# yangao07/abPOA

Measured on NVIDIA H100. Metric: GCUPS (DP cells/s), global/convex 10 kbp, higher is better.
Workload: dtype int16 (packed int16x2 DPX arithmetic; int32 kernel only as overflow fallback)

## Files before the change

### abpoa_b200/csrc/poa_kernels.cu

```cuda
#include <cuda_runtime.h>
#include <stdint.h>
#include <algorithm>
#include "poa_device.cuh"
#include "poa_chain.cuh"

#define FULL 0xffffffffu
#define NEG POA_NEG32

enum { LG = 0, AG = 1, CG = 2 };
enum { GLOBAL = 0, LOCAL = 1, EXTEND = 2 };

#define OP_M   0x1
#define OP_E1  0x2
#define OP_E2  0x4
#define OP_E   0x6
#define OP_F1  0x8
#define OP_F2  0x10
#define OP_F   0x18
#define OP_ALL 0x1f

__device__ __forceinline__ void ld8(const int16_t *p, int v[8]) {
    const uint4 u = *reinterpret_cast<const uint4 *>(p);
    v[0] = (int)(short)(u.x & 0xffff); v[1] = ((int)u.x) >> 16;
    v[2] = (int)(short)(u.y & 0xffff); v[3] = ((int)u.y) >> 16;
// ... 697 lines not shown
            int E1o[8], E2o[8];
            int lmax = NEG, lfirst = -1, llast = -1;
#pragma unroll
            for (int c = 0; c < 8; ++c) {
                const int j = g * 8 + c, jr = j - jbase;
                if (GAP == LG) {
                    x1 = max(x1, a1[c]);
                    int h = max(x1 - e1 * jr, NEG);
                    if (MODE == LOCAL) h = max(h, zr);
                    if (lgx) {
                        const int v = j >> xs;
                        const bool keep = active && j >= beg && j <= ((((end >> xs) + 1) << xs) - 1) &&
                                          (v <= lgx_v1 || (v == lgx_v1 + 1 && !(j & 1)));
                        H[c] = keep ? h : NEG;
                    } else
                    H[c] = inb[c] ? h : NEG;
                } else {
                    const int f1 = max(x1 - e1 * (jr - 1), NEG);
                    x1 = max(x1, a1[c]);
                    Fa[c] = f1;
                    if (GAP == AG) {
                        const int t = max(M[c], X1[c]);
                        int h = max(t, f1);
                        if (MODE == LOCAL) h = max(h, zr);
                        const bool from_t = (h == t);
                        E1o[c] = from_t ? max(X1[c] - e1, h - oe1) : (MODE == LOCAL ? 0 : NEG);
                        H[c] = h;
                    } else {
                        const int f2 = max(x2 - e2 * (jr - 1), NEG);
                        x2 = max(x2, a2[c]);
                        Fb[c] = f2;
                        int h = max(T[c], max(f1, f2));
                        if (MODE == LOCAL) h = max(h, zr);
                        int eo1 = max(X1[c] - e1, h - oe1), eo2 = max(X2[c] - e2, h - oe2);
                        if (MODE == LOCAL) { eo1 = max(eo1, zr); eo2 = max(eo2, zr); }
                        E1o[c] = eo1; E2o[c] = eo2; H[c] = h;
                    }
                    if (!inb[c]) { H[c] = NEG; E1o[c] = NEG; if (GAP == CG) E2o[c] = NEG; }
                }
                if (inb[c]) {
                    if (H[c] > lmax) { lmax = H[c]; lfirst = llast = j; }
                    else if (H[c] == lmax) llast = j;
                }
            }

            if (active) {
                const int rel = g - g0;
                if (rel < ring_groups) {
                    ST *rq = ringp + (size_t)rel * POA_GROUP;
                    st8(rq, H);
                    if (GAP != LG) st8(rq + ring_cells, E1o);
                    if (GAP == CG) st8(rq + 2 * ring_cells, E2o);
                }
                ST *q = rowp + (size_t)rel * POA_GROUP;
                st8(q, H);
                if (GAP != LG) { st8(q + (size_t)PL::E1 * ngrp * POA_GROUP, E1o); st8(q + (size_t)PL::F1 * ngrp * POA_GROUP, Fa); }
                if (GAP == CG) { st8(q + (size_t)PL::E2 * ngrp * POA_GROUP, E2o); st8(q + (size_t)PL::F2 * ngrp * POA_GROUP, Fb); }
            }

            if (banded || MODE != GLOBAL) {
                const int pm = __reduce_max_sync(FULL, lmax);
                const unsigned bm = __ballot_sync(FULL, lmax == pm && lfirst >= 0);
                if (bm) {
                    const int pl = __shfl_sync(FULL, lfirst, __ffs(bm) - 1);
                    const int pr = __shfl_sync(FULL, llast, 31 - __clz(bm));
                    if (pm > row_max) { row_max = pm; row_left = pl; row_right = pr; }
                    else if (pm == row_max) row_right = pr;
                }
            }
        }
        if (lane == 0) {
            PoaRowInfo ri; ri.beg = beg; ri.end = end; ri.left = row_left; ri.right = row_right;
            ring_info[i & rmask] = ri; ring_off[i & rmask] = my_off;
            rowinfo[i] = ri; { PoaRowOff z; z.off = my_off; z.p0 = mypred; *reinterpret_cast<uint2 *>(rowoff + i) = make_uint2(z.off, (unsigned)z.p0); }
        }
        if (MODE == LOCAL) {
            if (row_max > best_score) { best_score = row_max; best_i = i; best_j = row_left; }
        } else if (MODE == EXTEND) {
            if (row_max > best_score) { best_score = row_max; best_i = i; best_j = row_right; best_row = i; }
            else if (prm->zdrop > 0) {
                const int delta = jv.remain(best_row) - rem;
                if (best_score - row_max > prm->zdrop + e1 * abs(delta - (row_right - best_j))) stop = true;
            }
        }
        __syncwarp();
        }
        pb = pe; pe = n_pe; rbase = n_rbase; rem = n_rem; mypred = n_mypred; myps = n_myps;
    }

    if (MODE == GLOBAL) {
        const int sb = jv.predoff(n_rows - 1), sn = jv.predoff(n_rows) - sb;
        for (int k = 0; k < sn; ++k) {
            const int prow = jv.pred[sb + k];
            const PoaRowInfo pi = rowinfo[prow];
            const int endc = qlen > pi.end ? pi.end : qlen;
            const int pg0 = ((pi.beg >> xs) << xs) >> 3;
            const int v = (endc >= pi.beg) ? (int)planes[(size_t)rowoff[prow].off * POA_GROUP + (endc - pg0 * 8)] : NEG;
            if (v > best_score) { best_score = v; best_i = prow; best_j = endc; }
        }
    }
    res.best_score = best_score; res.best_i = best_i; res.best_j = best_j;
    res.cells = cells; res.max_band = max_band; res.plane_units_used = cursor;
    const long long clk1 = clock64();
    res.fwd_clk = clk1 - clk0;
    if (lane == 0) *jd.result = res;
    __syncwarp();
    if (prm->ret_cigar) {
        poa_backtrack<GAP, ST, MODE>(jv, jd, prm, mat_s, lane, best_i, best_j, *jd.result, xs);
        if (lane == 0) jd.result->bt_clk = clock64() - clk1;
    }
    if (lane == 0) signal_done(jd);
}

#ifdef POA_KPROF
#define KP_DECL long long kp[6] = {0,0,0,0,0,0}; long long kp_t = clock64(); int kdiag[4] = {0,0,0,0};
#define KP(n) { const long long t_ = clock64(); kp[n] += t_ - kp_t; kp_t = t_; }
#define KP_OUT(res) { for (int z_ = 0; z_ < 6; ++z_) (res).prof[z_] = kp[z_]; for (int z_ = 0; z_ < 4; ++z_) (res).diag[z_] = kdiag[z_]; }
#else
#define KP_DECL
#define KP(n)
#define KP_OUT(res)
#endif
#define NEGP (-30000)
#define NEGP2 0x8AD08AD0u

__device__ __forceinline__ unsigned pk(int lo, int hi) { return ((unsigned)lo & 0xffffu) | ((unsigned)hi << 16); }
__device__ __forceinline__ int lo16(unsigned v) { return (int)(short)(v & 0xffffu); }
__device__ __forceinline__ int hi16(unsigned v) { return ((int)v) >> 16; }
__device__ __forceinline__ unsigned bc_hi(unsigned v) { return __byte_perm(v, v, 0x3232); }
__device__ __forceinline__ unsigned sh1(unsigned prev, unsigned cur) { return __byte_perm(prev, cur, 0x5432); }

__device__ __forceinline__ void lane_excl_prefix(const unsigned a[4], unsigned xb, unsigned P[4]) {
    unsigned inc[4];
#pragma unroll
    for (int k = 0; k < 4; ++k) inc[k] = __vmaxs2(a[k], __byte_perm(a[k], NEGP2, 0x1054));
    inc[1] = __vmaxs2(inc[1], bc_hi(inc[0]));
    inc[2] = __vmaxs2(inc[2], bc_hi(inc[1]));
    inc[3] = __vmaxs2(inc[3], bc_hi(inc[2]));
    P[0] = __vmaxs2(sh1(xb, inc[0]), xb);
    P[1] = __vmaxs2(sh1(inc[0], inc[1]), xb);
    P[2] = __vmaxs2(sh1(inc[1], inc[2]), xb);
    P[3] = __vmaxs2(sh1(inc[2], inc[3]), xb);
}
__device__ __forceinline__ int lane_max8(const unsigned a[4]) {
    const unsigned m = __vmaxs2(__vmaxs2(a[0], a[1]), __vmaxs2(a[2], a[3]));
    return max(lo16(m), hi16(m));
}

struct P16Consts {
    unsigned K1[4], K2[4];
    unsigned KF1[4], KF2[4];
    unsigned KLG[4];
    unsigned NE1, NOE1, NE2, NOE2;
};
static inline unsigned pk_host(int lo, int hi) { return ((unsigned)lo & 0xffffu) | ((unsigned)hi << 16); }
static P16Consts make_p16_consts(int e1, int oe1, int e2, int oe2) {
    P16Consts c;
    for (int k = 0; k < 4; ++k) {
        c.K1[k] = pk_host(e1 * (2 * k), e1 * (2 * k + 1)); c.K2[k] = pk_host(e2 * (2 * k), e2 * (2 * k + 1));
        c.KF1[k] = pk_host(-(oe1 + e1 * (2 * k - 1)), -(oe1 + e1 * (2 * k))); c.KF2[k] = pk_host(-(oe2 + e2 * (2 * k - 1)), -(oe2 + e2 * (2 * k)));
        c.KLG[k] = pk_host(-e1 * (2 * k), -e1 * (2 * k + 1));
    }
    c.NE1 = pk_host(-e1, -e1); c.NOE1 = pk_host(-oe1, -oe1); c.NE2 = pk_host(-e2, -e2); c.NOE2 = pk_host(-oe2, -oe2);
    return c;
}

struct P16Smem {
    int *mat_s; uint4 *cap_lo, *cap_hi, *ring_meta; int16_t *ring_data;
};
__device__ __forceinline__ P16Smem p16_smem_init(uint8_t *dyn_smem, const PoaParamsDev *prm, int ring_rows, int lane) {
    P16Smem sm;
    sm.mat_s = reinterpret_cast<int *>(dyn_smem);
    sm.cap_lo = reinterpret_cast<uint4 *>(dyn_smem + POA_MAX_M * POA_MAX_M * sizeof(int));
    sm.cap_hi = sm.cap_lo + 9;
    sm.ring_meta = sm.cap_hi + 9;
    sm.ring_data = reinterpret_cast<int16_t *>(sm.ring_meta + ring_rows);
    const int m = prm->m;
    for (int t = lane; t < m * m; t += 32) sm.mat_s[t] = prm->mat[t];
    if (lane < 9) {
        unsigned lo[4], hi[4];
#pragma unroll
        for (int k = 0; k < 4; ++k) {
            lo[k] = pk(2 * k < lane ? NEGP : 32767, 2 * k + 1 < lane ? NEGP : 32767);
            hi[k] = pk(2 * k >= 8 - lane ? NEGP : 32767, 2 * k + 1 >= 8 - lane ? NEGP : 32767);
        }
        sm.cap_lo[lane] = make_uint4(lo[0], lo[1], lo[2], lo[3]);
        sm.cap_hi[lane] = make_uint4(hi[0], hi[1], hi[2], hi[3]);
    }
    __syncwarp();
    return sm;
}

template <int GAP, int MODE>
__device__ __forceinline__ void p16_cells(const P16Consts &kc, const unsigned CLO[4], const unsigned CAP[4], const unsigned S[4],
                                          unsigned M[4], const unsigned X1[4], const unsigned X2[4], int jr0, int e1, int oe1, int e2, int oe2,
                                          unsigned zr2, int lane, int &carry1, int &carry2,
                                          unsigned H[4], unsigned F1[4], unsigned F2[4], unsigned E1o[4], unsigned E2o[4]) {
    unsigned T[4];
#pragma unroll
    for (int k = 0; k < 4; ++k) {
        const unsigned hm = __viaddmax_s16x2(M[k], S[k], NEGP2);
        M[k] = __vmins2(hm, CLO[k]);
        if (GAP == LG) T[k] = __vmins2(__vmaxs2(hm, X1[k]), CLO[k]);
        else if (GAP == AG) T[k] = M[k];
        else T[k] = __vmins2(__vimax3_s16x2(hm, X1[k], X2[k]), CLO[k]);
    }
    unsigned a1[4], a2[4];
#pragma unroll
    for (int k = 0; k < 4; ++k) { a1[k] = __vadd2(T[k], kc.K1[k]); if (GAP == CG) a2[k] = __vadd2(T[k], kc.K2[k]); }
    const int off1 = e1 * jr0 - (GAP == LG ? 0 : oe1), off2 = e2 * jr0 - oe2;
    int tot1, tot2 = 0;
    int x1 = max(warp_excl_max(lane_max8(a1) + off1, lane, tot1), carry1);
    carry1 = max(carry1, tot1);
    const int xl1 = min(max(x1 - off1, NEGP), 32767);
    unsigned P1[4], P2[4];
    lane_excl_prefix(a1, pk(xl1, xl1), P1);
    if (GAP == CG) {
        int x2 = max(warp_excl_max(lane_max8(a2) + off2, lane, tot2), carry2);
        carry2 = max(carry2, tot2);
        const int xl2 = min(max(x2 - off2, NEGP), 32767);
        lane_excl_prefix(a2, pk(xl2, xl2), P2);
    }
#pragma unroll
    for (int k = 0; k < 4; ++k) {
        if (GAP == LG) {
            unsigned h = __viaddmax_s16x2(__vmaxs2(P1[k], a1[k]), kc.KLG[k], NEGP2);
            if (MODE == LOCAL) h = __vmaxs2(h, zr2);
            H[k] = __vmins2(h, CAP[k]);
        } else {
            F1[k] = __viaddmax_s16x2(P1[k], kc.KF1[k], NEGP2);
            if (GAP == AG) {
                const unsigned t = __vmaxs2(M[k], X1[k]);
                unsigned fz = F1[k];
                if (MODE == LOCAL) fz = __vmaxs2(fz, zr2);
                const unsigned h = __vmaxs2(t, fz);
                const unsigned from_t = __vcmpges2(t, fz);
                const unsigned ev = __viaddmax_s16x2(X1[k], kc.NE1, __viaddmax_s16x2(h, kc.NOE1, NEGP2));
                const unsigned alt = (MODE == LOCAL) ? zr2 : NEGP2;
                E1o[k] = __vmins2((ev & from_t) | (alt & ~from_t), CAP[k]);
                H[k] = __vmins2(h, CAP[k]);
            } else {
                F2[k] = __viaddmax_s16x2(P2[k], kc.KF2[k], NEGP2);
                unsigned h = __vimax3_s16x2(T[k], F1[k], F2[k]);
                if (MODE == LOCAL) h = __vmaxs2(h, zr2);
                unsigned eo1 = __viaddmax_s16x2(X1[k], kc.NE1, __viaddmax_s16x2(h, kc.NOE1, NEGP2));
                unsigned eo2 = __viaddmax_s16x2(X2[k], kc.NE2, __viaddmax_s16x2(h, kc.NOE2, NEGP2));
                if (MODE == LOCAL) { eo1 = __vmaxs2(eo1, zr2); eo2 = __vmaxs2(eo2, zr2); }
                H[k] = __vmins2(h, CAP[k]); E1o[k] = __vmins2(eo1, CAP[k]); E2o[k] = __vmins2(eo2, CAP[k]);
            }
        }
    }
}

template <int GAP>
__device__ __forceinline__ uint2 p16_fbits(const P16Consts &kc, const unsigned H[4], const unsigned F1[4], const unsigned F2[4],
                                           const unsigned CLO[4], const unsigned CAP[4], bool left_in, int lane, bool more,
                                           unsigned &lh, unsigned &lf1, unsigned &lf2) {
    const unsigned hl = __shfl_up_sync(FULL, H[3], 1), f1l = __shfl_up_sync(FULL, F1[3], 1);
    unsigned f2l = 0u;
    if (GAP == CG) f2l = __shfl_up_sync(FULL, F2[3], 1);
    const unsigned hp = lane == 0 ? lh : hl, f1p = lane == 0 ? lf1 : f1l, f2p = lane == 0 ? lf2 : f2l;
    const unsigned clp = left_in ? 0x7fff0000u : 0u;
    unsigned v[4];
#pragma unroll
    for (int k = 0; k < 4; ++k) {
        const unsigned inb = __vcmpeq2(CAP[k], 0x7fff7fffu);
        const unsigned inl = inb & __vcmpeq2(sh1(k ? CLO[k - 1] : clp, CLO[k]), 0x7fff7fffu);
        const unsigned hs = sh1(k ? H[k - 1] : hp, H[k]), fs1 = sh1(k ? F1[k - 1] : f1p, F1[k]);
        unsigned x = (__vcmpeq2(H[k], F1[k]) & inb & (FB_A * 0x10001u))
                   | (__vcmpeq2(__vadd2(hs, kc.NOE1), F1[k]) & inl & (FB_B * 0x10001u))
                   | (__vcmpeq2(__vadd2(fs1, kc.NE1), F1[k]) & inl & (FB_C * 0x10001u));
        if (GAP == CG) {
            const unsigned fs2 = sh1(k ? F2[k - 1] : f2p, F2[k]);
            x |= (__vcmpeq2(H[k], F2[k]) & inb & ((FB_A << 3) * 0x10001u))
               | (__vcmpeq2(__vadd2(hs, kc.NOE2), F2[k]) & inl & ((FB_B << 3) * 0x10001u))
               | (__vcmpeq2(__vadd2(fs2, kc.NE2), F2[k]) & inl & ((FB_C << 3) * 0x10001u));
        }
        v[k] = x;
    }
    if (more) {
        lh = __shfl_sync(FULL, H[3], 31); lf1 = __shfl_sync(FULL, F1[3], 31);
        if (GAP == CG) lf2 = __shfl_sync(FULL, F2[3], 31);
    }
    return make_uint2(__byte_perm(v[0], v[1], 0x6420), __byte_perm(v[2], v[3], 0x6420));
}

template <int GAP, int MODE, bool DUMP>
__device__ int fb_recompute(const JobView &jv, const PoaJobDesc &jd, const PoaParamsDev *prm, const FbCtx &fx,
                            int beg, int end, int pb, int np, int base, int j, int lane) {
    const P16Consts &kc = *fx.kc;
    const int16_t *planes = reinterpret_cast<const int16_t *>(jd.planes);
    const int e1 = prm->e1, oe1 = prm->oe1, e2 = prm->e2, oe2 = prm->oe2;
    const unsigned zr2 = (unsigned)prm->zero;
    const int qstride = ((jv.qlen + 1 + 7) & ~7) + 8;
    const int16_t *qrow = jd.qprof + (size_t)base * qstride;
    const int g0 = beg >> 3, g1 = end >> 3;
    const int pj = ((j >> 3) - g0) >> 5;
    const int p_lo = max(0, pj - max(fx.buf_cells >> 8, 1) + 1);
    const int lo = (g0 + 32 * p_lo) * 8;
    int carry1 = 2 * NEG, carry2 = 2 * NEG;
    unsigned lh = 0u, lf1 = 0u, lf2 = 0u;
    for (int p = 0; p <= pj; ++p) {
        const int gp = g0 + 32 * p, g = gp + lane;
        const bool active = g <= g1;
        uint4 sv = make_uint4(0u, 0u, 0u, 0u);
        if (active) sv = *reinterpret_cast<const uint4 *>(qrow + (size_t)g * 8);
        unsigned M[4], X1[4], X2[4];
#pragma unroll
        for (int k = 0; k < 4; ++k) { M[k] = NEGP2; X1[k] = NEGP2; X2[k] = NEGP2; }
        const bool fix_left = (gp > g0) || ((beg & 7) == 0);
        for (int kb = 0; kb < np; kb += 32) {
            int c_g0 = 0, c_ng = 0; uint32_t c_off = 0;
            if (kb + lane < np) {
                const int prow = ldb(jv.pred + pb + kb + lane);
                const PoaRowInfo pi = jd.rowinfo[prow];
                c_g0 = pi.beg >> 3; c_ng = (pi.end >> 3) - c_g0 + 1; c_off = jd.rowoff[prow].off;
            }
            const int nk = min(32, np - kb);
            for (int k = 0; k < nk; ++k) {
                const int pg0 = __shfl_sync(FULL, c_g0, k), png = __shfl_sync(FULL, c_ng, k);
                const uint32_t off = __shfl_sync(FULL, c_off, k);
                const int16_t *ph = planes + (size_t)off * POA_GROUP;
                const size_t pp = (size_t)png * POA_GROUP;
                const int rel = g - pg0;
                uint4 hp = make_uint4(NEGP2, NEGP2, NEGP2, NEGP2), ep1 = hp, ep2 = hp;
                if (active && (unsigned)rel < (unsigned)png) {
                    const int16_t *q = ph + (size_t)rel * POA_GROUP;
                    hp = *reinterpret_cast<const uint4 *>(q);
                    if (GAP != LG) ep1 = *reinterpret_cast<const uint4 *>(q + (size_t)Planes<GAP>::E1 * pp);
                    if (GAP == CG) ep2 = *reinterpret_cast<const uint4 *>(q + (size_t)Planes<GAP>::E2 * pp);
                }
                unsigned prev = __shfl_up_sync(FULL, hp.w, 1);
                if (lane == 0) {
                    int hm1 = NEGP;
                    if (fix_left && (unsigned)(rel - 1) < (unsigned)png) hm1 = (int)ph[(size_t)(rel - 1) * POA_GROUP + 7];
                    if (MODE == LOCAL && g == 0) hm1 = 0;
                    prev = (unsigned)hm1 << 16;
                }
                M[0] = __vmaxs2(M[0], sh1(prev, hp.x)); M[1] = __vmaxs2(M[1], sh1(hp.x, hp.y));
                M[2] = __vmaxs2(M[2], sh1(hp.y, hp.z)); M[3] = __vmaxs2(M[3], sh1(hp.z, hp.w));
                X1[0] = __vmaxs2(X1[0], ep1.x); X1[1] = __vmaxs2(X1[1], ep1.y); X1[2] = __vmaxs2(X1[2], ep1.z); X1[3] = __vmaxs2(X1[3], ep1.w);
                if (GAP == CG) { X2[0] = __vmaxs2(X2[0], ep2.x); X2[1] = __vmaxs2(X2[1], ep2.y); X2[2] = __vmaxs2(X2[2], ep2.z); X2[3] = __vmaxs2(X2[3], ep2.w); }
            }
        }
        const int nlo = min(max(beg - g * 8, 0), 8), nhi = min(max(g * 8 + 7 - end, 0), 8);
        const uint4 clo = fx.cap_lo[nlo], chi = fx.cap_hi[nhi];
        const unsigned CLO[4] = { clo.x, clo.y, clo.z, clo.w };
        const unsigned CAP[4] = { __vmins2(clo.x, chi.x), __vmins2(clo.y, chi.y), __vmins2(clo.z, chi.z), __vmins2(clo.w, chi.w) };
        const unsigned S[4] = { sv.x, sv.y, sv.z, sv.w };
        unsigned H[4], F1[4], F2[4], E1o[4], E2o[4];
        p16_cells<GAP, MODE>(kc, CLO, CAP, S, M, X1, X2, (g - g0) * 8, e1, oe1, e2, oe2, zr2, lane, carry1, carry2, H, F1, F2, E1o, E2o);
        const uint2 bits = p16_fbits<GAP>(kc, H, F1, F2, CLO, CAP, g > g0, lane, p < pj, lh, lf1, lf2);
        if (p >= p_lo && active) *reinterpret_cast<uint2 *>(fx.buf + (g * 8 - lo)) = bits;
        if constexpr (DUMP) {
            if (p >= p_lo && active) {
                const FbDumpCtx &dx = static_cast<const FbDumpCtx &>(fx);
                int16_t *q = dx.f + (size_t)(g - g0) * POA_GROUP;
                *reinterpret_cast<uint4 *>(q) = make_uint4(F1[0], F1[1], F1[2], F1[3]);
                if (GAP == CG) *reinterpret_cast<uint4 *>(q + dx.fstride) = make_uint4(F2[0], F2[1], F2[2], F2[3]);
            }
        }
    }
    __syncwarp();
    return lo;
}

template <int GAP, int MODE, bool LEAN = false, bool TMA = false, bool FB = false>
__device__ __forceinline__ void p16_run_job(const PoaJobDesc &jd, const PoaParamsDev *__restrict__ prm, const P16Consts &kc, const P16Smem &sm,
                                            int ring_rows, int ring_cells, int lane) {
    static_assert(!(TMA && FB), "the TMA row drain stages the five-plane layout");
    typedef int16_t ST;
    typedef Planes<GAP> PL;
    typedef RowLayout<GAP, FB> RL;
    constexpr int RN = RingPlanes<GAP>::N;
    int *mat_s = sm.mat_s; uint4 *cap_lo = sm.cap_lo, *cap_hi = sm.cap_hi, *ring_meta = sm.ring_meta; ST *ring_data = sm.ring_data;
    const int rmask = ring_rows - 1, ring_groups = ring_cells >> 3;
    const long long clk0 = clock64();
    uint64_t t_start_ns; asm volatile("mov.u64 %0, %%globaltimer;" : "=l"(t_start_ns));
    const int m = prm->m;
    const JobView jv = open_job(jd.blob);
    ST *planes = reinterpret_cast<ST *>(jd.planes);
    PoaRowInfo *rowinfo = jd.rowinfo; PoaRowOff *rowoff = jd.rowoff;
    const int qlen = jv.qlen, n_rows = jv.n_rows, w = jv.w;
    const bool banded = w >= 0;
    const int e1 = prm->e1, o1 = prm->o1, oe1 = prm->oe1, e2 = prm->e2, o2 = prm->o2, oe2 = prm->oe2;
    const int pnv = jv.pn;
    const unsigned zr2 = (unsigned)prm->zero;

    PoaResultDev res;
    res.status = POA_ST_OK; res.best_score = NEG; res.best_i = 0; res.best_j = 0; res.n_ops = 0;
    res.start_i = res.start_j = 0; res.n_aln_bases = res.n_matched_bases = 0; res.max_band = 0; res.cells = 0; res.plane_units_used = 0;
    res.fwd_clk = 0; res.bt_clk = 0; res.t_start_ns = t_start_ns; res.t_end_ns = 0;

    int16_t *qp = jd.qprof;
    const int qstride = ((qlen + 1 + 7) & ~7) + 8;
    for (int r = 0; r < m; ++r)
        for (int j = lane; j < qstride; j += 32)
            qp[(size_t)r * qstride + j] = (j == 0 || j > qlen) ? (int16_t)0 : (int16_t)mat_s[r * m + jv.qs[j]];
    __syncwarp();

    uint64_t cursor = 0;
    int64_t cells = 0; int max_band = 0;
    int best_score = NEG, best_i = 0, best_j = 0, best_row = 0;
    int guard_lo = 0, guard_hi = 0;
    bool stop = false;

    {
        int end0 = qlen;
        if (banded) end0 = min(qlen, max(0, qlen - jv.remain(0)) + w);
        const int g1 = end0 >> 3, ngrp = g1 + 1;
        if ((uint64_t)RL::units(ngrp) > jd.plane_cap_units) { if (lane == 0) { res.status = POA_ST_PLANE_OVF; *jd.result = res; } return; }
        for (int gp = 0; gp <= g1; gp += 32) {
            const int g = gp + lane;
            if (g <= g1) {
                int h[8], ea[8], eb[8], fa[8], fb[8];
#pragma unroll
                for (int c = 0; c < 8; ++c) {
                    const int j = g * 8 + c;
                    if (MODE == LOCAL) { h[c] = ea[c] = eb[c] = fa[c] = fb[c] = (j <= end0) ? 0 : NEGP; }
                    else if (j > end0) { h[c] = ea[c] = eb[c] = fa[c] = fb[c] = NEGP; }
                    else if (GAP == LG) { h[c] = max(-e1 * j, NEGP); }
                    else if (j == 0) { h[c] = 0; ea[c] = -oe1; eb[c] = -oe2; fa[c] = fb[c] = NEGP; }
                    else {
                        fa[c] = max(-o1 - e1 * j, NEGP); fb[c] = max(-o2 - e2 * j, NEGP); ea[c] = eb[c] = NEGP;
                        h[c] = (GAP == CG) ? max(fa[c], fb[c]) : fa[c];
                    }
                }
                ST *rp = planes + (size_t)g * POA_GROUP;
                st8(rp, h);
                if (GAP != LG) st8(rp + (size_t)PL::E1 * ngrp * POA_GROUP, ea);
                if (GAP == CG) st8(rp + (size_t)PL::E2 * ngrp * POA_GROUP, eb);
                if (!FB && GAP != LG) st8(rp + (size_t)PL::F1 * ngrp * POA_GROUP, fa);
                if (!FB && GAP == CG) st8(rp + (size_t)PL::F2 * ngrp * POA_GROUP, fb);
                if (g < ring_groups) {
                    ST *rq = ring_data + (size_t)g * POA_GROUP;
                    st8(rq, h);
                    if (GAP != LG) st8(rq + ring_cells, ea);
                    if (GAP == CG) st8(rq + 2 * ring_cells, eb);
                }
            }
        }
        if (lane == 0) {
            PoaRowInfo r0; r0.beg = 0; r0.end = end0; r0.left = 0; r0.right = 0;
            rowinfo[0] = r0; { PoaRowOff z; z.off = 0; z.p0 = -1; rowoff[0] = z; } ring_meta[0] = make_uint4(0u, (unsigned)end0, 1u | (1u << 16), 0u);
        }
        cursor = RL::units(ngrp);
        cells += end0 + 1; max_band = end0 + 1;
        __syncwarp();
    }

    const uint32_t ring_s = (uint32_t)__cvta_generic_to_shared(ring_data);
    constexpr int RS = TMA ? PL::N : RN;
    const uint32_t ring_row_bytes = (uint32_t)(RS * ring_cells * 2), ring_plane_bytes = (uint32_t)(ring_cells * 2);
    const int pn_shift = pnv == 16 ? 4 : 3;
    const uint32_t cap32 = jd.plane_cap_units > 0xffffffffull ? 0xffffffffu : (uint32_t)jd.plane_cap_units;
    uint32_t cur32 = (uint32_t)cursor;
    const bool has_ps = LEAN ? false : (jv.predscore != nullptr);

    const int npred_tot = ldb(&jv.rowmeta[n_rows].x);
    int pb = 0, pe = 0, rbase = 0, rem = 0, raw_pred = -1, raw_ps = 0;
    if (n_rows > 2) {
        { const int2 m1 = ldb(jv.rowmeta + 1); pb = m1.x; pe = jv.predoff(2); rbase = m1.y & 0xff; rem = m1.y >> 8; }
        { const int k = max(min(pb + lane, npred_tot - 1), 0); raw_pred = ldb(jv.pred + k); if (has_ps) raw_ps = ldb(jv.predscore + k); }
    }
    int nx_y = n_rows > 3 ? ldb(&jv.rowmeta[2].y) : 0;
    constexpr int LP = 4;
    int lp_c[LP];
#pragma unroll
    for (int k = 0; k < LP; ++k) lp_c[k] = LEAN ? __shfl_sync(FULL, lane < pe - pb ? raw_pred : -1, k) : -1;
    KP_DECL
    for (int i = 1; i < n_rows - 1 && !stop; ++i) {
        KP(5)
        const int np = pe - pb;
        const int mypred = lane < np ? raw_pred : -1, myps = lane < np ? raw_ps : 0;
        int lp[LP];
#pragma unroll
        for (int k = 0; k < LP; ++k) lp[k] = lp_c[k];
        int2 m2;
        m2.x = ldb(&jv.rowmeta[i + 2].x); m2.y = ldb(&jv.rowmeta[i + 2].y);
        const int n_rbase = nx_y & 0xff, n_rem = nx_y >> 8;
        int n_raw_pred, n_raw_ps = 0;
        { const int k = max(min(pe + lane, npred_tot - 1), 0); n_raw_pred = ldb(jv.pred + k); if (has_ps) n_raw_ps = ldb(jv.predscore + k); }
        if (LEAN || !(jv.live && !ldb(jv.live + i))) {

        bool lean_row = false;
        uint4 lm[LP];
#pragma unroll
        for (int k = 0; k < LP; ++k) lm[k] = make_uint4(0u, 0u, 0u, 0u);
        if (LEAN) {
            lean_row = np >= 1 && np <= LP;
#pragma unroll
            for (int k = 0; k < LP; ++k) if (k < np && (i - lp[k]) > rmask) lean_row = false;
#ifdef POA_KPROF
            if (!lean_row) { if (np > LP || np < 1) ++kdiag[1]; else ++kdiag[2]; }
#endif
            if (lean_row) {
                lm[0] = ring_meta[lp[0] & rmask];
                int wide = (int)(lm[0].y >> 3) - (int)(lm[0].x >> 3) + 1;
#pragma unroll
                for (int k = 1; k < LP; ++k) {
                    lm[k] = k < np ? ring_meta[lp[k] & rmask] : lm[0];
                    wide = max(wide, (int)(lm[k].y >> 3) - (int)(lm[k].x >> 3) + 1);
                }
                if (wide > ring_groups) lean_row = false;
#ifdef POA_KPROF
                if (lean_row) ++kdiag[0]; else ++kdiag[3];
#endif
            }
        }
        unsigned wA = 0, wB = 0;
        int l1 = INT32_MAX, r1 = INT32_MIN, b1 = INT32_MAX;
        if (!lean_row && lane < np) {
            const int prow = mypred;
            const bool near = (i - prow) <= rmask;
            uint4 mi;
            if (near) mi = ring_meta[prow & rmask];
            else { const PoaRowInfo pi = rowinfo[prow]; mi = make_uint4((unsigned)pi.beg, (unsigned)pi.end, (unsigned)(pi.left + 1) | ((unsigned)(pi.right + 1) << 16), rowoff[prow].off); }
            l1 = (int)(mi.z & 0xffffu); r1 = (int)(mi.z >> 16); b1 = (int)mi.x;
            const unsigned pg0 = mi.x >> 3, png = (mi.y >> 3) - pg0 + 1;
            wA = pg0 | (png << 12) | ((unsigned)near << 25) | ((unsigned)(prow & rmask) << 26);
            wB = mi.w;
        }
        int ml = jv.node_n, mr = 0, min_pre_beg = INT32_MAX;
        if (lean_row) {
#pragma unroll
            for (int k = 0; k < LP; ++k) {
                ml = min(ml, (int)(lm[k].z & 0xffffu)); mr = max(mr, (int)(lm[k].z >> 16)); min_pre_beg = min(min_pre_beg, (int)lm[k].x);
            }
        } else if (banded) {
            ml = min(ml, __reduce_min_sync(FULL, l1));
            mr = max(mr, __reduce_max_sync(FULL, r1));
            min_pre_beg = __reduce_min_sync(FULL, b1);
            for (int kb = 32; kb < np; kb += 32) {
                const int k = kb + lane;
                int l2 = INT32_MAX, r2 = INT32_MIN, b2 = INT32_MAX;
                if (k < np) { const PoaRowInfo pi = rowinfo[ldb(jv.pred + pb + k)]; l2 = pi.left + 1; r2 = pi.right + 1; b2 = pi.beg; }
                ml = min(ml, __reduce_min_sync(FULL, l2)); mr = max(mr, __reduce_max_sync(FULL, r2)); min_pre_beg = min(min_pre_beg, __reduce_min_sync(FULL, b2));
            }
        }
        int beg = 0, end = qlen;
        if (banded) {
            const int r = qlen - rem;
            beg = max(0, min(ml, r) - w);
            end = min(qlen, max(mr, r) + w);
            if (np > 0 && (beg >> pn_shift) < (min_pre_beg >> pn_shift)) beg = min_pre_beg;
        }
        const int g0 = beg >> 3, g1 = end >> 3, ngrp = g1 - g0 + 1;
        const uint32_t need = RL::units((uint32_t)ngrp);
        if (need > cap32 - cur32) {
            if (TMA) { if (lane == 0) asm volatile("cp.async.bulk.wait_group 0;" ::: "memory"); __syncwarp(); }
            if (lane == 0) { res.status = POA_ST_PLANE_OVF; res.plane_units_used = cur32; *jd.result = res; }
            return;
        }
        const bool tma_row = TMA && ngrp <= ring_groups;
        const uint32_t my_off = cur32;
        cur32 += need;
        ST *rowp = planes + (size_t)my_off * POA_GROUP;
        const size_t gplane = (size_t)ngrp * POA_GROUP;
        const uint32_t my_ring_s = ring_s + (uint32_t)(i & rmask) * ring_row_bytes;
        cells += (end >= beg) ? (end - beg + 1) : 0;
        max_band = max(max_band, end - beg + 1);
        const int16_t *qrow = qp + (size_t)rbase * qstride;
        if (i + 1 < n_rows - 1) {
            const int16_t *nrow = qp + (size_t)n_rbase * qstride;
            const int c0 = min((g0 + lane) * 8, qstride - 8);
            asm volatile("prefetch.global.L1 [%0];" :: "l"(nrow + c0));
            if (lane >= 24) asm volatile("prefetch.global.L1 [%0];" :: "l"(nrow + min(c0 + 64, qstride - 8)));
        }

        int carry1 = 2 * NEG, carry2 = 2 * NEG;
        int row_max = NEG, row_left = -1, row_right = -1;
        KP(0)

        for (int gp = g0; gp <= g1; gp += 32) {
            const int g = gp + lane;
            const bool active = g <= g1;
            uint4 sv = make_uint4(0u, 0u, 0u, 0u);
            if (active) sv = *reinterpret_cast<const uint4 *>(qrow + (size_t)g * 8);
            unsigned M[4], X1[4], X2[4];
            unsigned D0[4];
#pragma unroll
            for (int k = 0; k < 4; ++k) { M[k] = NEGP2; X1[k] = NEGP2; X2[k] = NEGP2; D0[k] = NEGP2; }
            const bool fix_left = (gp > g0) || ((beg & 7) == 0);

            if (lean_row) {
#pragma unroll
                for (int k = 0; k < LP; ++k) {
                    if (k >= np) break;
                    const uint4 mi = lm[k];
                    const int pg0 = (int)(mi.x >> 3), png = (int)(mi.y >> 3) - pg0 + 1;
                    const int rel = g - pg0;
                    const bool inr = active && (unsigned)rel < (unsigned)png;
                    const uint32_t prs = ring_s + (uint32_t)(lp[k] & rmask) * ring_row_bytes;
                    uint4 hp = make_uint4(NEGP2, NEGP2, NEGP2, NEGP2), ep1 = hp, ep2 = hp;
                    if (inr) {
                        const uint32_t a = prs + (uint32_t)rel * 16u;
                        asm volatile("ld.shared.v4.u32 {%0,%1,%2,%3}, [%4];" : "=r"(hp.x), "=r"(hp.y), "=r"(hp.z), "=r"(hp.w) : "r"(a));
                        if (GAP != LG) asm volatile("ld.shared.v4.u32 {%0,%1,%2,%3}, [%4];" : "=r"(ep1.x), "=r"(ep1.y), "=r"(ep1.z), "=r"(ep1.w) : "r"(a + ring_plane_bytes));
                        if (GAP == CG) asm volatile("ld.shared.v4.u32 {%0,%1,%2,%3}, [%4];" : "=r"(ep2.x), "=r"(ep2.y), "=r"(ep2.z), "=r"(ep2.w) : "r"(a + 2 * ring_plane_bytes));
                    }
                    unsigned prev = __shfl_up_sync(FULL, hp.w, 1);
                    if (fix_left) {
                        if (lane == 0) {
                            int hm1 = NEGP;
                            const int relm = rel - 1;
                            if ((unsigned)relm < (unsigned)png) { unsigned short v; asm volatile("ld.shared.u16 %0, [%1];" : "=h"(v) : "r"(prs + (uint32_t)relm * 16u + 14u)); hm1 = (int)(short)v; }
                            if (MODE == LOCAL && g == 0) hm1 = 0;
                            prev = (unsigned)hm1 << 16;
                        }
                    } else if (lane == 0) prev = (MODE == LOCAL && g == 0) ? 0u : ((unsigned)NEGP << 16);
                    const unsigned d0 = sh1(prev, hp.x), d1 = sh1(hp.x, hp.y), d2 = sh1(hp.y, hp.z), d3 = sh1(hp.z, hp.w);
                    if (GAP == LG) {
                        hp.x = __viaddmax_s16x2(hp.x, kc.NE1, NEGP2); hp.y = __viaddmax_s16x2(hp.y, kc.NE1, NEGP2); hp.z = __viaddmax_s16x2(hp.z, kc.NE1, NEGP2); hp.w = __viaddmax_s16x2(hp.w, kc.NE1, NEGP2);
                    }
                    const uint4 x1 = GAP == LG ? hp : ep1;
                    if (k == 0) {
                        D0[0] = d0; D0[1] = d1; D0[2] = d2; D0[3] = d3;
                        M[0] = d0; M[1] = d1; M[2] = d2; M[3] = d3;
                        X1[0] = x1.x; X1[1] = x1.y; X1[2] = x1.z; X1[3] = x1.w;
                        if (GAP == CG) { X2[0] = ep2.x; X2[1] = ep2.y; X2[2] = ep2.z; X2[3] = ep2.w; }
                    } else {
                        M[0] = __vmaxs2(M[0], d0); M[1] = __vmaxs2(M[1], d1); M[2] = __vmaxs2(M[2], d2); M[3] = __vmaxs2(M[3], d3);
                        X1[0] = __vmaxs2(X1[0], x1.x); X1[1] = __vmaxs2(X1[1], x1.y); X1[2] = __vmaxs2(X1[2], x1.z); X1[3] = __vmaxs2(X1[3], x1.w);
                        if (GAP == CG) { X2[0] = __vmaxs2(X2[0], ep2.x); X2[1] = __vmaxs2(X2[1], ep2.y); X2[2] = __vmaxs2(X2[2], ep2.z); X2[3] = __vmaxs2(X2[3], ep2.w); }
                    }
                }
            } else
            for (int kb = 0; kb < np; kb += 32) {
                unsigned cA = wA, cB = wB; int c_ps = myps;
                if (kb > 0) {
                    const int k = kb + lane; cA = 0; cB = 0; c_ps = 0;
                    if (k < np) {
                        const int prow = ldb(jv.pred + pb + k); const PoaRowInfo pi = rowinfo[prow];
                        const unsigned pg0 = (unsigned)pi.beg >> 3, png = ((unsigned)pi.end >> 3) - pg0 + 1;
                        cA = pg0 | (png << 12); cB = rowoff[prow].off; if (has_ps) c_ps = ldb(jv.predscore + pb + k);
                    }
                }
                const int nk = min(32, np - kb);
                for (int k = 0; k < nk; ++k) {
                    const unsigned A = __shfl_sync(FULL, cA, k), B = __shfl_sync(FULL, cB, k);
                    const int pg0 = (int)(A & 0xfffu), png = (int)((A >> 12) & 0x1fffu);
                    const bool near = (A >> 25) & 1u;
                    const int rel = g - pg0;
                    const bool inr = active && (unsigned)rel < (unsigned)png;
                    uint4 hp = make_uint4(NEGP2, NEGP2, NEGP2, NEGP2), ep1 = hp, ep2 = hp;
                    const uint32_t prs = ring_s + (A >> 26) * ring_row_bytes;
                    const ST *ph = planes + (size_t)B * POA_GROUP;
                    if (inr) {
                        if (near && rel < ring_groups) {
                            const uint32_t a = prs + (uint32_t)rel * 16u;
                            asm volatile("ld.shared.v4.u32 {%0,%1,%2,%3}, [%4];" : "=r"(hp.x), "=r"(hp.y), "=r"(hp.z), "=r"(hp.w) : "r"(a));
                            if (GAP != LG) asm volatile("ld.shared.v4.u32 {%0,%1,%2,%3}, [%4];" : "=r"(ep1.x), "=r"(ep1.y), "=r"(ep1.z), "=r"(ep1.w) : "r"(a + ring_plane_bytes));
                            if (GAP == CG) asm volatile("ld.shared.v4.u32 {%0,%1,%2,%3}, [%4];" : "=r"(ep2.x), "=r"(ep2.y), "=r"(ep2.z), "=r"(ep2.w) : "r"(a + 2 * ring_plane_bytes));
                        } else {
                            const ST *q = ph + (size_t)rel * POA_GROUP;
                            const size_t pp = (size_t)png * POA_GROUP;
                            hp = *reinterpret_cast<const uint4 *>(q);
                            if (GAP != LG) ep1 = *reinterpret_cast<const uint4 *>(q + (size_t)PL::E1 * pp);
                            if (GAP == CG) ep2 = *reinterpret_cast<const uint4 *>(q + (size_t)PL::E2 * pp);
                        }
                    }
                    unsigned prev = __shfl_up_sync(FULL, hp.w, 1);
                    if (lane == 0) {
                        int hm1 = NEGP;
                        if (fix_left) {
                            const int relm = rel - 1;
                            if ((unsigned)relm < (unsigned)png) {
                                if (near && relm < ring_groups) { unsigned short v; asm volatile("ld.shared.u16 %0, [%1];" : "=h"(v) : "r"(prs + (uint32_t)relm * 16u + 14u)); hm1 = (int)(short)v; }
                                else hm1 = (int)ph[(size_t)relm * POA_GROUP + 7];
                            }
                        }
                        if (MODE == LOCAL && g == 0) hm1 = 0;
                        prev = (unsigned)hm1 << 16;
                    }
                    unsigned d0 = sh1(prev, hp.x), d1 = sh1(hp.x, hp.y), d2 = sh1(hp.y, hp.z), d3 = sh1(hp.z, hp.w);
                    if (has_ps) {
                        const int ps = __shfl_sync(FULL, c_ps, k);
                        const unsigned ps2 = pk(ps, ps);
                        d0 = __viaddmax_s16x2(d0, ps2, NEGP2); d1 = __viaddmax_s16x2(d1, ps2, NEGP2);
                        d2 = __viaddmax_s16x2(d2, ps2, NEGP2); d3 = __viaddmax_s16x2(d3, ps2, NEGP2);
                        if (GAP == LG) {
                            hp.x = __viaddmax_s16x2(hp.x, ps2, NEGP2); hp.y = __viaddmax_s16x2(hp.y, ps2, NEGP2);
                            hp.z = __viaddmax_s16x2(hp.z, ps2, NEGP2); hp.w = __viaddmax_s16x2(hp.w, ps2, NEGP2);
                        } else {
                            ep1.x = __viaddmax_s16x2(ep1.x, ps2, NEGP2); ep1.y = __viaddmax_s16x2(ep1.y, ps2, NEGP2);
                            ep1.z = __viaddmax_s16x2(ep1.z, ps2, NEGP2); ep1.w = __viaddmax_s16x2(ep1.w, ps2, NEGP2);
                            if (GAP == CG) {
                                ep2.x = __viaddmax_s16x2(ep2.x, ps2, NEGP2); ep2.y = __viaddmax_s16x2(ep2.y, ps2, NEGP2);
                                ep2.z = __viaddmax_s16x2(ep2.z, ps2, NEGP2); ep2.w = __viaddmax_s16x2(ep2.w, ps2, NEGP2);
                            }
                        }
                    }
                    if (kb == 0 && k == 0) { D0[0] = d0; D0[1] = d1; D0[2] = d2; D0[3] = d3; }
                    M[0] = __vmaxs2(M[0], d0); M[1] = __vmaxs2(M[1], d1); M[2] = __vmaxs2(M[2], d2); M[3] = __vmaxs2(M[3], d3);
                    if (GAP == LG) {
                        X1[0] = __vmaxs2(X1[0], __viaddmax_s16x2(hp.x, kc.NE1, NEGP2)); X1[1] = __vmaxs2(X1[1], __viaddmax_s16x2(hp.y, kc.NE1, NEGP2));
                        X1[2] = __vmaxs2(X1[2], __viaddmax_s16x2(hp.z, kc.NE1, NEGP2)); X1[3] = __vmaxs2(X1[3], __viaddmax_s16x2(hp.w, kc.NE1, NEGP2));
                    } else {
                        X1[0] = __vmaxs2(X1[0], ep1.x); X1[1] = __vmaxs2(X1[1], ep1.y); X1[2] = __vmaxs2(X1[2], ep1.z); X1[3] = __vmaxs2(X1[3], ep1.w);
                        if (GAP == CG) { X2[0] = __vmaxs2(X2[0], ep2.x); X2[1] = __vmaxs2(X2[1], ep2.y); X2[2] = __vmaxs2(X2[2], ep2.z); X2[3] = __vmaxs2(X2[3], ep2.w); }
                    }
                }
            }

            KP(1)
            const int nlo = min(max(beg - g * 8, 0), 8), nhi = min(max(g * 8 + 7 - end, 0), 8);
            const uint4 clo = cap_lo[nlo], chi = cap_hi[nhi];
            const unsigned CLO[4] = { clo.x, clo.y, clo.z, clo.w };
            const unsigned CAP[4] = { __vmins2(clo.x, chi.x), __vmins2(clo.y, chi.y), __vmins2(clo.z, chi.z), __vmins2(clo.w, chi.w) };
            const unsigned S[4] = { sv.x, sv.y, sv.z, sv.w };

            unsigned H[4], F1[4], F2[4], E1o[4], E2o[4];
            p16_cells<GAP, MODE>(kc, CLO, CAP, S, M, X1, X2, (g - g0) * 8, e1, oe1, e2, oe2, zr2, lane, carry1, carry2, H, F1, F2, E1o, E2o);

            if (jd.btrec != nullptr) {
                unsigned t = 0;
#pragma unroll
                for (int k = 0; k < 4; ++k)
                    t |= __vcmpeq2(__viaddmax_s16x2(D0[k], S[k], NEGP2), H[k]) & (0x00020001u << (2 * k));
                const unsigned byte = (t | (t >> 16)) & 0xffu;
                uint8_t *rec = reinterpret_cast<uint8_t *>(jd.btrec + i);
                const int rel = g - g0;
                if (active && rel < POA_BTREC_GROUPS) rec[16 + rel] = (uint8_t)byte;
                if (lane == 0 && gp == g0)
                    *reinterpret_cast<uint4 *>(rec) = make_uint4((unsigned)(g0 * 8), (unsigned)mypred,
                                                                 (unsigned)rbase | (ngrp <= POA_BTREC_GROUPS ? 0x100u : 0u) | ((unsigned)min(ngrp, 0xffff) << 16), (unsigned)my_off);
            }
            KP(2)
            if (TMA && tma_row) {
                if (gp == g0) {
                    if (lane == 0) { if (ring_rows >= 8) asm volatile("cp.async.bulk.wait_group.read 7;" ::: "memory"); else asm volatile("cp.async.bulk.wait_group.read 0;" ::: "memory"); }
                    __syncwarp();
                }
                if (active) {
                    const uint32_t a = my_ring_s + (uint32_t)(g - g0) * 16u;
                    asm volatile("st.shared.v4.u32 [%0], {%1,%2,%3,%4};" :: "r"(a), "r"(H[0]), "r"(H[1]), "r"(H[2]), "r"(H[3]) : "memory");
                    if (GAP != LG) {
                        asm volatile("st.shared.v4.u32 [%0], {%1,%2,%3,%4};" :: "r"(a + (uint32_t)PL::E1 * ring_plane_bytes), "r"(E1o[0]), "r"(E1o[1]), "r"(E1o[2]), "r"(E1o[3]) : "memory");
                        asm volatile("st.shared.v4.u32 [%0], {%1,%2,%3,%4};" :: "r"(a + (uint32_t)PL::F1 * ring_plane_bytes), "r"(F1[0]), "r"(F1[1]), "r"(F1[2]), "r"(F1[3]) : "memory");
                    }
                    if (GAP == CG) {
                        asm volatile("st.shared.v4.u32 [%0], {%1,%2,%3,%4};" :: "r"(a + (uint32_t)PL::E2 * ring_plane_bytes), "r"(E2o[0]), "r"(E2o[1]), "r"(E2o[2]), "r"(E2o[3]) : "memory");
                        asm volatile("st.shared.v4.u32 [%0], {%1,%2,%3,%4};" :: "r"(a + (uint32_t)PL::F2 * ring_plane_bytes), "r"(F2[0]), "r"(F2[1]), "r"(F2[2]), "r"(F2[3]) : "memory");
                    }
                }
            } else
            if (active) {
                const int rel = g - g0;
                if (rel < ring_groups) {
                    const uint32_t a = my_ring_s + (uint32_t)rel * 16u;
                    asm volatile("st.shared.v4.u32 [%0], {%1,%2,%3,%4};" :: "r"(a), "r"(H[0]), "r"(H[1]), "r"(H[2]), "r"(H[3]) : "memory");
                    if (GAP != LG) asm volatile("st.shared.v4.u32 [%0], {%1,%2,%3,%4};" :: "r"(a + ring_plane_bytes), "r"(E1o[0]), "r"(E1o[1]), "r"(E1o[2]), "r"(E1o[3]) : "memory");
                    if (GAP == CG) asm volatile("st.shared.v4.u32 [%0], {%1,%2,%3,%4};" :: "r"(a + 2 * ring_plane_bytes), "r"(E2o[0]), "r"(E2o[1]), "r"(E2o[2]), "r"(E2o[3]) : "memory");
                }
                ST *q = rowp + (size_t)rel * POA_GROUP;
                *reinterpret_cast<uint4 *>(q) = make_uint4(H[0], H[1], H[2], H[3]);
                if (GAP != LG) *reinterpret_cast<uint4 *>(q + (size_t)PL::E1 * gplane) = make_uint4(E1o[0], E1o[1], E1o[2], E1o[3]);
                if (GAP == CG) *reinterpret_cast<uint4 *>(q + (size_t)PL::E2 * gplane) = make_uint4(E2o[0], E2o[1], E2o[2], E2o[3]);
                if (!FB && GAP != LG) *reinterpret_cast<uint4 *>(q + (size_t)PL::F1 * gplane) = make_uint4(F1[0], F1[1], F1[2], F1[3]);
                if (!FB && GAP == CG) *reinterpret_cast<uint4 *>(q + (size_t)PL::F2 * gplane) = make_uint4(F2[0], F2[1], F2[2], F2[3]);
            }

            KP(3)
            {
                const int lmax = active ? lane_max8(H) : NEGP;
                unsigned eq = 0;
#pragma unroll
                for (int k = 0; k < 4; ++k) { eq |= (unsigned)(lo16(H[k]) == lmax) << (2 * k); eq |= (unsigned)(hi16(H[k]) == lmax) << (2 * k + 1); }
                const int lfirst = g * 8 + __ffs(eq) - 1, llast = g * 8 + 31 - __clz(eq);
                const int pm = __reduce_max_sync(FULL, lmax);
                const unsigned bm = __ballot_sync(FULL, lmax == pm && pm > NEGP);
                if (bm) {
                    const int pl = __shfl_sync(FULL, lfirst, __ffs(bm) - 1);
                    const int pr = __shfl_sync(FULL, llast, 31 - __clz(bm));
                    if (pm > row_max) { row_max = pm; row_left = pl; row_right = pr; }
                    else if (pm == row_max) row_right = pr;
                }
            }
        }
        KP(4)
        if (TMA && tma_row) {
            asm volatile("fence.proxy.async.shared::cta;" ::: "memory");
            __syncwarp();
            if (lane == 0) {
                const uint32_t bytes = (uint32_t)ngrp * 16u;
#pragma unroll
                for (int pl = 0; pl < PL::N; ++pl)
                    asm volatile("cp.async.bulk.global.shared::cta.bulk_group [%0], [%1], %2;"
                                 :: "l"(rowp + (size_t)pl * gplane), "r"(my_ring_s + (uint32_t)pl * ring_plane_bytes), "r"(bytes) : "memory");
                asm volatile("cp.async.bulk.commit_group;" ::: "memory");
            }
        }
        if (lane == 0) {
            ring_meta[i & rmask] = make_uint4((unsigned)beg, (unsigned)end, (unsigned)(row_left + 1) | ((unsigned)(row_right + 1) << 16), my_off);
            PoaRowInfo ri; ri.beg = beg; ri.end = end; ri.left = row_left; ri.right = row_right;
            rowinfo[i] = ri; { PoaRowOff z; z.off = my_off; z.p0 = mypred; *reinterpret_cast<uint2 *>(rowoff + i) = make_uint2(z.off, (unsigned)z.p0); }
        }
        guard_lo |= (row_max < -14000); guard_hi |= (row_max > 29000);
        if (MODE == LOCAL) {
            if (row_max > best_score) { best_score = row_max; best_i = i; best_j = row_left; }
        } else if (MODE == EXTEND) {
            if (row_max > best_score) { best_score = row_max; best_i = i; best_j = row_right; best_row = i; }
            else if (prm->zdrop > 0) {
                const int delta = jv.remain(best_row) - rem;
                if (best_score - row_max > prm->zdrop + e1 * abs(delta - (row_right - best_j))) stop = true;
            }
        }
        __syncwarp();
        }
        asm volatile("" : "+r"(m2.x), "+r"(m2.y), "+r"(n_raw_pred), "+r"(n_raw_ps));
        pb = pe; pe = m2.x; rbase = n_rbase; rem = n_rem; nx_y = m2.y; raw_pred = n_raw_pred; raw_ps = n_raw_ps;
#pragma unroll
        for (int k = 0; k < LP; ++k) lp_c[k] = LEAN ? __shfl_sync(FULL, lane < pe - pb ? raw_pred : -1, k) : -1;
    }
    cursor = cur32;
    KP_OUT(res)
    if (TMA) {
        if (lane == 0) asm volatile("cp.async.bulk.wait_group 0;" ::: "memory");
        __syncwarp();
    }

    if (MODE == GLOBAL) {
        const int sb = jv.predoff(n_rows - 1), sn = jv.predoff(n_rows) - sb;
        for (int k = 0; k < sn; ++k) {
            const int prow = jv.pred[sb + k];
            const PoaRowInfo pi = rowinfo[prow];
            const int endc = qlen > pi.end ? pi.end : qlen;
            const int pg0 = pi.beg >> 3;
            const int v = (endc >= pi.beg) ? (int)planes[(size_t)rowoff[prow].off * POA_GROUP + (endc - pg0 * 8)] : NEG;
            if (v > best_score) { best_score = v; best_i = prow; best_j = endc; }
        }
    }
    res.best_score = best_score; res.best_i = best_i; res.best_j = best_j;
    res.cells = cells; res.max_band = max_band; res.plane_units_used = cursor;
    if (guard_lo || guard_hi || best_score <= NEGP + 2000) res.status = POA_ST_RANGE;
    if (banded && MODE != LOCAL && (int64_t)max_band * max(e1, e2) + max(oe1, oe2) > 15000) res.status = POA_ST_RANGE;
    const long long clk1 = clock64();
    res.fwd_clk = clk1 - clk0;
#ifndef POA_KPROF
    { unsigned smid; asm volatile("mov.u32 %0, %%smid;" : "=r"(smid)); res.prof[5] = (int64_t)smid; }
#endif
    if (lane == 0) *jd.result = res;
    __syncwarp();
    if (prm->ret_cigar && res.status == POA_ST_OK) {
        FbCtx fx;
        fx.kc = &kc; fx.cap_lo = cap_lo; fx.cap_hi = cap_hi;
        fx.buf = reinterpret_cast<uint8_t *>(ring_data); fx.buf_cells = (int)ring_row_bytes * ring_rows;
        poa_backtrack<GAP, ST, MODE, FB>(jv, jd, prm, mat_s, lane, best_i, best_j, *jd.result, 3, jd.btrec, &fx);
        if (lane == 0) jd.result->bt_clk = clock64() - clk1;
    }
}


#ifndef POA_P16_MINB
#define POA_P16_MINB 10
#endif
#define POA_P16_BOUNDS __launch_bounds__(32, POA_P16_MINB)
template <int GAP, int MODE, bool LEAN, bool TMA>
__global__ void POA_P16_BOUNDS poa_align_kernel_p16(const PoaJobDesc *__restrict__ jobs, const PoaParamsDev *__restrict__ prm,
                                                           int n_jobs, int ring_rows, int ring_cells, const __grid_constant__ P16Consts kc) {
    extern __shared__ __align__(16) uint8_t dyn_smem[];
    const int lane = threadIdx.x;
    const int job = blockIdx.x;
    if (job >= n_jobs) return;
    const P16Smem sm = p16_smem_init(dyn_smem, prm, ring_rows, lane);
    const PoaJobDesc jd = jobs[job];
    p16_run_job<GAP, MODE, LEAN, TMA>(jd, prm, kc, sm, ring_rows, ring_cells, lane);
    __syncwarp();
    if (lane == 0) signal_done(jd);
}

static inline size_t ring_smem_bytes(int gap, int bits, int ring_rows, int ring_cells, int all_planes = 0);

template <int GAP>
__global__ void POA_P16_BOUNDS poa_chain_align_kernel_p16(const PoaChainSlot *__restrict__ slots, const int32_t *__restrict__ idx,
                                                           const PoaParamsDev *__restrict__ prm, int n_jobs, int round, int ring_rows, int ring_cells,
                                                           const __grid_constant__ P16Consts kc) {
    extern __shared__ __align__(16) uint8_t dyn_smem[];
    const int lane = threadIdx.x;
    const int job = blockIdx.x;
    if (job >= n_jobs) return;
    const PoaChainSlot *sl = &slots[idx[job]];
    if (job == 0 && lane == 0 && sl->pool_cursor) sl->pool_cursor[(round + 1) & 1] = 0ull;
    const PoaJobDesc jd = sl->jd;
    const int n_rows = reinterpret_cast<const PoaJobHeader *>(jd.blob)->n_rows;
    if (sl->failed || sl->fused >= sl->n_reads || n_rows < 3) { if (lane == 0) jd.result->status = POA_ST_SKIP; return; }
    const P16Smem sm = p16_smem_init(dyn_smem, prm, ring_rows, lane);
    p16_run_job<GAP, GLOBAL, true, false, true>(jd, prm, kc, sm, ring_rows, ring_cells, lane);
}

__device__ __forceinline__ int chain_ld_relaxed(const int32_t *p) { int v; asm volatile("ld.relaxed.gpu.global.s32 %0, [%1];" : "=r"(v) : "l"(p) : "memory"); return v; }
__device__ __forceinline__ void chain_st_relaxed(int32_t *p, int v) { asm volatile("st.relaxed.gpu.global.s32 [%0], %1;" :: "l"(p), "r"(v) : "memory"); }
__device__ __forceinline__ unsigned long long chain_now_ns() { unsigned long long t; asm volatile("mov.u64 %0, %%globaltimer;" : "=l"(t)); return t; }

template <int GAP>
__global__ void POA_P16_BOUNDS poa_chain_dp_worker_kernel(PoaChainSlot *slots, PoaChainSync *sync, const PoaParamsDev *__restrict__ prm, int n_groups,
                                                          int ring_rows, int ring_cells, int dbg, const __grid_constant__ P16Consts kc) {
    extern __shared__ __align__(16) uint8_t dyn_smem[];
    const int lane = threadIdx.x;
    const int g = blockIdx.x;
    if (g >= n_groups) return;
    PoaChainSlot *sl = &slots[g];
    const P16Smem sm = p16_smem_init(dyn_smem, prm, ring_rows, lane);
    const unsigned long long limit = sync->watchdog_ns;
    int pushed = 0;
    unsigned long long waited = 0;
    for (;;) {
        int state = 0;
        {
            const unsigned long long t0 = chain_now_ns();
            unsigned ns = 500, polls = 0;
            for (;;) {
                const int v = __shfl_sync(0xffffffffu, chain_ld_relaxed(&sl->turn), 0);
                if (v == 0) break;
                __nanosleep(ns); if (ns < 8000) ns <<= 1;
                if ((++polls & 63u) == 0) {
                    const int a = __shfl_sync(0xffffffffu, chain_ld_relaxed(&sync->abort), 0);
                    const unsigned late = __shfl_sync(0xffffffffu, (unsigned)(chain_now_ns() - t0 > limit), 0);
                    if (a) { state = 2; break; }
                    if (late) { if (lane == 0) chain_st_relaxed(&sync->abort, 1); state = 2; break; }
                }
// ... 228 lines not shown
```

Baseline: 126.5.

## Use packed int16x2 shuffle scan for F gap prefix across the warp

Replaces the per-row int32 warp exclusive max scan of the F (vertical gap) prefix with a packed int16x2 shuffle scan. It runs both gap planes in one register and adds a decayed per-step penalty using viaddmax, with the carry kept in packed form. The new path is enabled only when the gap extension costs are small enough to avoid int16 saturation, otherwise the old int32 path runs. The row max and argmax computation is also vectorised with packed compares instead of per-halfword scalar comparisons. This cuts shuffle and ALU instructions on the critical per-row path, at the risk of precision differences in the saturating int16 scan.

```diff
diff --git a/abpoa_b200/csrc/poa_kernels.cu b/abpoa_b200/csrc/poa_kernels.cu
--- a/abpoa_b200/csrc/poa_kernels.cu
+++ b/abpoa_b200/csrc/poa_kernels.cu
@@ -873,7 +873,10 @@
     unsigned KF1[4], KF2[4];
     unsigned KLG[4];
     unsigned NE1, NOE1, NE2, NOE2;
+    unsigned KS[5];
+    int pscan;
 };
+#define P16_PSCAN_MAX_E 21
 static inline unsigned pk_host(int lo, int hi) { return ((unsigned)lo & 0xffffu) | ((unsigned)hi << 16); }
 static P16Consts make_p16_consts(int e1, int oe1, int e2, int oe2) {
     P16Consts c;
@@ -883,6 +886,8 @@
         c.KLG[k] = pk_host(-e1 * (2 * k), -e1 * (2 * k + 1));
     }
     c.NE1 = pk_host(-e1, -e1); c.NOE1 = pk_host(-oe1, -oe1); c.NE2 = pk_host(-e2, -e2); c.NOE2 = pk_host(-oe2, -oe2);
+    for (int s = 0; s < 5; ++s) c.KS[s] = pk_host(-8 * e1 * (1 << s), -8 * e2 * (1 << s));
+    c.pscan = e1 <= P16_PSCAN_MAX_E && e2 <= P16_PSCAN_MAX_E;
     return c;
 }
 
@@ -912,10 +917,25 @@
     return sm;
 }
 
+struct FCarry {
+    int c1 = 2 * NEG, c2 = 2 * NEG;
+    unsigned p = NEGP2;
+};
+
+__device__ __forceinline__ unsigned p16_fscan(const P16Consts &kc, unsigned m, int lane, unsigned &carry) {
+    if (lane == 0) m = __viaddmax_s16x2(carry, kc.KS[0], m);
+#pragma unroll
+    for (int s = 0; s < 5; ++s) m = __viaddmax_s16x2(__shfl_up_sync(FULL, m, 1 << s), kc.KS[s], m);
+    unsigned t = __shfl_up_sync(FULL, m, 1);
+    if (lane == 0) t = carry;
+    carry = __shfl_sync(FULL, m, 31);
+    return __viaddmax_s16x2(t, kc.KS[0], NEGP2);
+}
+
 template <int GAP, int MODE>
 __device__ __forceinline__ void p16_cells(const P16Consts &kc, const unsigned CLO[4], const unsigned CAP[4], const unsigned S[4],
                                           unsigned M[4], const unsigned X1[4], const unsigned X2[4], int jr0, int e1, int oe1, int e2, int oe2,
-                                          unsigned zr2, int lane, int &carry1, int &carry2,
+                                          unsigned zr2, int lane, FCarry &fc,
                                           unsigned H[4], unsigned F1[4], unsigned F2[4], unsigned E1o[4], unsigned E2o[4]) {
     unsigned T[4];
 #pragma unroll
@@ -929,18 +949,30 @@
     unsigned a1[4], a2[4];
 #pragma unroll
     for (int k = 0; k < 4; ++k) { a1[k] = __vadd2(T[k], kc.K1[k]); if (GAP == CG) a2[k] = __vadd2(T[k], kc.K2[k]); }
-    const int off1 = e1 * jr0 - (GAP == LG ? 0 : oe1), off2 = e2 * jr0 - oe2;
-    int tot1, tot2 = 0;
-    int x1 = max(warp_excl_max(lane_max8(a1) + off1, lane, tot1), carry1);
-    carry1 = max(carry1, tot1);
-    const int xl1 = min(max(x1 - off1, NEGP), 32767);
     unsigned P1[4], P2[4];
-    lane_excl_prefix(a1, pk(xl1, xl1), P1);
-    if (GAP == CG) {
-        int x2 = max(warp_excl_max(lane_max8(a2) + off2, lane, tot2), carry2);
-        carry2 = max(carry2, tot2);
-        const int xl2 = min(max(x2 - off2, NEGP), 32767);
-        lane_excl_prefix(a2, pk(xl2, xl2), P2);
+    if (kc.pscan) {
+        const unsigned m1 = __vmaxs2(__vmaxs2(a1[0], a1[1]), __vmaxs2(a1[2], a1[3]));
+        unsigned m;
+        if (GAP == CG) {
+            const unsigned m2 = __vmaxs2(__vmaxs2(a2[0], a2[1]), __vmaxs2(a2[2], a2[3]));
+            m = __vmaxs2(__byte_perm(m1, m2, 0x5410), __byte_perm(m1, m2, 0x7632));
+        } else m = __vmaxs2(m1, __byte_perm(m1, m1, 0x1032));
+        const unsigned x = p16_fscan(kc, m, lane, fc.p);
+        lane_excl_prefix(a1, __byte_perm(x, x, 0x1010), P1);
+        if (GAP == CG) lane_excl_prefix(a2, bc_hi(x), P2);
+    } else {
+        const int off1 = e1 * jr0 - (GAP == LG ? 0 : oe1), off2 = e2 * jr0 - oe2;
+        int tot1, tot2 = 0;
+        int x1 = max(warp_excl_max(lane_max8(a1) + off1, lane, tot1), fc.c1);
+        fc.c1 = max(fc.c1, tot1);
+        const int xl1 = min(max(x1 - off1, NEGP), 32767);
+        lane_excl_prefix(a1, pk(xl1, xl1), P1);
+        if (GAP == CG) {
+            int x2 = max(warp_excl_max(lane_max8(a2) + off2, lane, tot2), fc.c2);
+            fc.c2 = max(fc.c2, tot2);
+            const int xl2 = min(max(x2 - off2, NEGP), 32767);
+            lane_excl_prefix(a2, pk(xl2, xl2), P2);
+        }
     }
 #pragma unroll
     for (int k = 0; k < 4; ++k) {
@@ -1019,7 +1051,7 @@
     const int pj = ((j >> 3) - g0) >> 5;
     const int p_lo = max(0, pj - max(fx.buf_cells >> 8, 1) + 1);
     const int lo = (g0 + 32 * p_lo) * 8;
-    int carry1 = 2 * NEG, carry2 = 2 * NEG;
+    FCarry fc;
     unsigned lh = 0u, lf1 = 0u, lf2 = 0u;
     for (int p = 0; p <= pj; ++p) {
         const int gp = g0 + 32 * p, g = gp + lane;
@@ -1070,7 +1102,7 @@
         const unsigned CAP[4] = { __vmins2(clo.x, chi.x), __vmins2(clo.y, chi.y), __vmins2(clo.z, chi.z), __vmins2(clo.w, chi.w) };
         const unsigned S[4] = { sv.x, sv.y, sv.z, sv.w };
         unsigned H[4], F1[4], F2[4], E1o[4], E2o[4];
-        p16_cells<GAP, MODE>(kc, CLO, CAP, S, M, X1, X2, (g - g0) * 8, e1, oe1, e2, oe2, zr2, lane, carry1, carry2, H, F1, F2, E1o, E2o);
+        p16_cells<GAP, MODE>(kc, CLO, CAP, S, M, X1, X2, (g - g0) * 8, e1, oe1, e2, oe2, zr2, lane, fc, H, F1, F2, E1o, E2o);
         const uint2 bits = p16_fbits<GAP>(kc, H, F1, F2, CLO, CAP, g > g0, lane, p < pj, lh, lf1, lf2);
         if (p >= p_lo && active) *reinterpret_cast<uint2 *>(fx.buf + (g * 8 - lo)) = bits;
         if constexpr (DUMP) {
@@ -1289,7 +1321,7 @@
             if (lane >= 24) asm volatile("prefetch.global.L1 [%0];" :: "l"(nrow + min(c0 + 64, qstride - 8)));
         }
 
-        int carry1 = 2 * NEG, carry2 = 2 * NEG;
+        FCarry fc;
         int row_max = NEG, row_left = -1, row_right = -1;
         KP(0)
 
@@ -1432,7 +1464,7 @@
             const unsigned S[4] = { sv.x, sv.y, sv.z, sv.w };
 
             unsigned H[4], F1[4], F2[4], E1o[4], E2o[4];
-            p16_cells<GAP, MODE>(kc, CLO, CAP, S, M, X1, X2, (g - g0) * 8, e1, oe1, e2, oe2, zr2, lane, carry1, carry2, H, F1, F2, E1o, E2o);
+            p16_cells<GAP, MODE>(kc, CLO, CAP, S, M, X1, X2, (g - g0) * 8, e1, oe1, e2, oe2, zr2, lane, fc, H, F1, F2, E1o, E2o);
 
             if (jd.btrec != nullptr) {
                 unsigned t = 0;
@@ -1484,10 +1516,13 @@
 
             KP(3)
             {
-                const int lmax = active ? lane_max8(H) : NEGP;
-                unsigned eq = 0;
-#pragma unroll
-                for (int k = 0; k < 4; ++k) { eq |= (unsigned)(lo16(H[k]) == lmax) << (2 * k); eq |= (unsigned)(hi16(H[k]) == lmax) << (2 * k + 1); }
+                const unsigned hm = __vmaxs2(__vmaxs2(H[0], H[1]), __vmaxs2(H[2], H[3]));
+                const unsigned lm2 = __vmaxs2(hm, __byte_perm(hm, hm, 0x1032));
+                const int lmax = active ? lo16(lm2) : NEGP;
+                unsigned t = 0;
+#pragma unroll
+                for (int k = 0; k < 4; ++k) t |= __vcmpeq2(H[k], lm2) & (0x00020001u << (2 * k));
+                const unsigned eq = (t | (t >> 16)) & 0xffu;
                 const int lfirst = g * 8 + __ffs(eq) - 1, llast = g * 8 + 31 - __clz(eq);
                 const int pm = __reduce_max_sync(FULL, lmax);
                 const unsigned bm = __ballot_sync(FULL, lmax == pm && pm > NEGP);
```

After: 127.9, median of 6. +1.1%, better.
